# vga-group/tauray

Hardware: AMD Instinct MI355X
Metric: Mray/s (closest-hit + shadow rays traced) @1920x1080, 4 bounces, 1 spp (higher is better)
Workload: dtype f32

## Files before the change

tauray_amd/csrc/api.hip:

```cpp
#include <cstdlib>
#include <cstring>
#include <mutex>
#include <string>
#include <vector>

#include "pt.h"
#include "trace.h"
#include "trace_quad.h"
#include "specialize.h"
#include "tonemap.h"
#include "../../include/tauray_image.hh"
#include "../../include/tauray_exr.hh"

namespace tr {

static thread_local std::string g_error;
int set_error(const std::string& msg) { g_error = msg; return 1; }

#define HIPCHK(x) do { hipError_t e_ = (x); if (e_ != hipSuccess) return set_error(std::string(#x) + ": " + hipGetErrorString(e_)); } while (0)

namespace {

constexpr int KB = TR_BLOCK;

// ... 119 lines not shown
                if (lh.light >= 0) out[ri] = HitRecord{-1, lh.light, lh.t, 0.0f, lh.t};
            }
        }
    }
    if (overflow) *overflow_flag = 1;
}
__global__ __launch_bounds__(KB) void k_query_terminal(SceneView sv, uint n, const float* rays, const uint* seeds, const uint* fallback, HitRecord* out, uint* overflow_flag,
                                                       int* qspill) {
    __shared__ int s_stack_rows[TR_STACK_WORDS];
    int* const s_stack = s_stack_rows + TR_STACK_ROW0;
    __shared__ int s_owner[(KB / 64) * TR_OWNER_WORDS];
    int* my_stack = s_stack + threadIdx.x;
    QuadCtx qc;
    qc.wave_stack = s_stack + (threadIdx.x & ~63u);
    qc.owner_tab = s_owner + (threadIdx.x >> 6) * TR_OWNER_WORDS;
    qc.spill = qspill + ((size_t)blockIdx.x * (KB / 64) + (threadIdx.x >> 6)) * (16u * TR_QSPILL);
    int overflow = 0;
    TraceStats st = {};
    for (uint base = blockIdx.x * KB; base < n; base += gridDim.x * KB) {
        const uint i = base + threadIdx.x;
        const bool valid = i < n;
        float r[8] = {0, 0, 0, 0, 0, 0, 0, 0};
        if (valid) for (int k = 0; k < 8; ++k) r[k] = rays[(size_t)i * 8 + k];
        const uint seed = (valid && seeds) ? seeds[i] : 0u;
        TerminalRay term = {valid && !(fallback && fallback[i] != 0u), false};
        HitRecord hit;
        if (seeds) trace_closest_wave4<0, false, false, true>(sv, valid, F3(r[0], r[1], r[2]), F3(r[4], r[5], r[6]), r[3], r[7], seed, my_stack, qc, hit, st, overflow, &term);
        else trace_closest_wave4<1, false, false, true>(sv, valid, F3(r[0], r[1], r[2]), F3(r[4], r[5], r[6]), r[3], r[7], 0u, my_stack, qc, hit, st, overflow, &term);
        if (valid) out[i] = term.blocked ? HitRecord{TR_HIT_BLOCKED, -1, 0.0f, 0.0f, -1.0f} : hit;
    }
    if (overflow) *overflow_flag = 1;
}
template <bool TWO_LEVEL>
__global__ __launch_bounds__(KB) void k_query_shadow(SceneView sv, uint n, const float* rays, float* out, uint* overflow_flag) {
    __shared__ int s_stack_rows[TR_STACK_WORDS];
    int* const s_stack = s_stack_rows + TR_STACK_ROW0;
    int overflow = 0;
    TraceStats st = {};
    for (uint i = blockIdx.x * KB + threadIdx.x; i < n; i += gridDim.x * KB) {
        const float* r = rays + (size_t)i * 8;
        out[i] = trace_shadow4<false, TWO_LEVEL>(sv, F3(r[0], r[1], r[2]), F3(r[4], r[5], r[6]), r[3], r[7], s_stack + threadIdx.x, st, overflow);
    }
    if (overflow) *overflow_flag = 1;
}

__global__ __launch_bounds__(KB) void k_stitch(LaunchCtx L, const f4* partial, uint pw, uint ph, f4* primary, uint viewports, float blend_ratio) {
    uint per_view = L.strategy == 2 ? L.launch_w : pw * ph;
    uint i = blockIdx.x * KB + threadIdx.x;
    if (i >= per_view * viewports) return;
    uint z = i / per_view, p = i % per_view;
    uint sx, sy, ox, oy;
    if (L.strategy == 2) {
        uint j = permute_region_id(L.index + p, L.size_x, L.size_y, L.count);
        if (j >= L.size_x * L.size_y) return;
        sx = p % L.size_x; sy = p / L.size_x;
        ox = j % L.size_x; oy = j / L.size_x;
    } else {
        sx = p % pw; sy = p / pw;
        ox = sx; oy = sy * L.count + L.index;
        if (oy >= L.size_y) return;
    }
    f4 c = partial[((size_t)z * ph + sy) * pw + sx];
    size_t o = ((size_t)z * L.size_y + oy) * L.size_x + ox;
    if (blend_ratio < 1.0f) c = mix4(primary[o], c, blend_ratio);
    primary[o] = c;
}

#define TR_STITCH_BATCH 15
struct StitchBatch { LaunchCtx L[TR_STITCH_BATCH]; const f4* partial[TR_STITCH_BATCH]; uint pw[TR_STITCH_BATCH], ph[TR_STITCH_BATCH]; };
__global__ __launch_bounds__(KB) void k_stitch_batch(StitchBatch B, f4* primary, uint viewports, float blend_ratio) {
    const uint e = blockIdx.y;
    const LaunchCtx L = B.L[e];
    const uint pw = B.pw[e], ph = B.ph[e];
    const f4* partial = B.partial[e];
// ... 14 lines not shown
    }
    f4 c = partial[((size_t)z * ph + sy) * pw + sx];
    size_t o = ((size_t)z * L.size_y + oy) * L.size_x + ox;
    if (blend_ratio < 1.0f) c = mix4(primary[o], c, blend_ratio);
    primary[o] = c;
}

__global__ __launch_bounds__(KB) void k_tonemap(const f4* in, f4* out, uint w, uint h, uint layers, int op, float exposure, float gamma, int grid) {
    size_t i = (size_t)blockIdx.x * KB + threadIdx.x;
    size_t n = (size_t)w * h * layers;
    if (i >= n) return;
    out[i] = tonemap_pixel(in[i], op, exposure, gamma, grid, (uint)(i % w), (uint)((i / w) % h));
}

template <typename T>
int upload_array(T*& dst, const void* src, size_t count) {
    dst = nullptr;
    if (count == 0 || !src) return 0;
    HIPCHK(hipMalloc(&dst, count * sizeof(T)));
    HIPCHK(hipMemcpy(dst, src, count * sizeof(T), hipMemcpyHostToDevice));
    return 0;
}

}
}

using namespace tr;

struct trhip_device {
    int hip_device = 0;
    DeviceScene scene;
    uint* overflow_flag = nullptr;
    int* qspill = nullptr;
};
constexpr uint QUERY_BLOCKS = 2048;
struct trhip_pt {
    trhip_device* dev;
    PtStage* stage;
};

namespace tr { int device_index(const trhip_device* dev) { return dev ? dev->hip_device : -1; } }
namespace tr { DeviceScene* device_scene(trhip_device* dev) { return dev ? &dev->scene : nullptr; } }
namespace tr { uint* device_overflow_flag(trhip_device* dev) { return dev ? dev->overflow_flag : nullptr; } }

#define DEVCHK(dev) do { if (!(dev)) return set_error("null trhip_device"); hipError_t e_ = hipSetDevice((dev)->hip_device); \
    if (e_ != hipSuccess) return set_error(std::string("hipSetDevice: ") + hipGetErrorString(e_)); } while (0)

extern "C" {

const char* trhip_last_error(void) { return g_error.c_str(); }

int trhip_image_decode(const void* data, size_t bytes, uint32_t* width, uint32_t* height, uint32_t* channels_in_file, uint8_t** rgba_out) {
    if (!data || !width || !height || !rgba_out) return set_error("trhip_image_decode: null argument");
    try {
        tr::image::decoded d = tr::image::decode(static_cast<const uint8_t*>(data), bytes);
        uint8_t* p = static_cast<uint8_t*>(malloc(d.rgba.size() ? d.rgba.size() : 1));
        if (!p) return set_error("trhip_image_decode: out of memory");
        memcpy(p, d.rgba.data(), d.rgba.size());
        *width = d.w; *height = d.h; *rgba_out = p;
        if (channels_in_file) *channels_in_file = (uint32_t)d.channels_in_file;
    } catch (const std::exception& e) { return set_error(e.what()); }
    return 0;
}
int trhip_image_decode_texels(const void* data, size_t bytes, uint32_t* width, uint32_t* height, uint32_t* channels_in_file, uint32_t* bits, uint8_t** texels_out) {
    if (!data || !width || !height || !bits || !texels_out) return set_error("trhip_image_decode_texels: null argument");
    try {
// ... 28 lines not shown
    try {
        const std::vector<uint8_t> b = tr::exr::encode(rgba, width, height, alpha != 0, half != 0, compression);
        uint8_t* p = static_cast<uint8_t*>(malloc(b.size()));
        if (!p) return set_error("trhip_exr_encode: out of memory");
        memcpy(p, b.data(), b.size());
        *bytes_out = p; *size_out = b.size();
    } catch (const std::exception& e) { return set_error(e.what()); }
    return 0;
}
void trhip_exr_free(void* p) { free(p); }

int trhip_device_create(int hip_device, trhip_device** out) {
    if (!out) return set_error("trhip_device_create: null out");
    int count = 0;
    hipError_t e = hipGetDeviceCount(&count);
    if (e != hipSuccess || count == 0) return set_error(std::string("trhip_device_create: no HIP device available (") + hipGetErrorString(e) + ")");
    if (hip_device < 0 || hip_device >= count) return set_error("trhip_device_create: device index out of range");
    HIPCHK(hipSetDevice(hip_device));
    trhip_device* d = new trhip_device();
    d->hip_device = hip_device;
    HIPCHK(hipMalloc(&d->overflow_flag, 4));
    HIPCHK(hipMemset(d->overflow_flag, 0, 4));
    { int cls = -1; (void)stream_pool_class(nullptr, &cls, true); }
    *out = d;
    return 0;
}
void trhip_device_destroy(trhip_device* dev) {
    if (!dev) return;
    (void)hipSetDevice(dev->hip_device);
    (void)hipDeviceSynchronize();
    dev->scene.free_all();
    if (dev->overflow_flag) (void)hipFree(dev->overflow_flag);
    if (dev->qspill) (void)hipFree(dev->qspill);
    delete dev;
}
int trhip_malloc(trhip_device* dev, size_t bytes, void** out) { DEVCHK(dev); HIPCHK(hipMalloc(out, bytes ? bytes : 16)); return 0; }
int trhip_free(trhip_device* dev, void* ptr) { DEVCHK(dev); if (ptr) HIPCHK(hipFree(ptr)); return 0; }
int trhip_upload(trhip_device* dev, void* dst, const void* src, size_t bytes, void* stream) {
    DEVCHK(dev); HIPCHK(hipMemcpyAsync(dst, src, bytes, hipMemcpyHostToDevice, (hipStream_t)stream)); HIPCHK(hipStreamSynchronize((hipStream_t)stream)); return 0;
}
int trhip_download(trhip_device* dev, void* dst, const void* src, size_t bytes, void* stream) {
    DEVCHK(dev); HIPCHK(hipMemcpyAsync(dst, src, bytes, hipMemcpyDeviceToHost, (hipStream_t)stream)); HIPCHK(hipStreamSynchronize((hipStream_t)stream)); return 0;
}
int trhip_memset(trhip_device* dev, void* dst, int value, size_t bytes, void* stream) { DEVCHK(dev); HIPCHK(hipMemsetAsync(dst, value, bytes, (hipStream_t)stream)); return 0; }
int trhip_sync(trhip_device* dev, void* stream) { DEVCHK(dev); HIPCHK(hipStreamSynchronize((hipStream_t)stream)); return 0; }
int trhip_stream_create(trhip_device* dev, void** stream_out) {
    DEVCHK(dev);
    if (!stream_out) return set_error("trhip_stream_create: null argument");
    hipStream_t st = nullptr;
    if (int rc = stream_pool_acquire(&st)) return rc;
    *stream_out = st;
    return 0;
}
int trhip_stream_destroy(trhip_device* dev, void* stream) {
    DEVCHK(dev);
    if (stream) { HIPCHK(hipStreamSynchronize((hipStream_t)stream)); stream_pool_release((hipStream_t)stream); }
    return 0;
}
int trhip_stream_pipe_class(trhip_device* dev, void* stream, int32_t* pipe_class_out) {
    DEVCHK(dev);
    if (!pipe_class_out) return set_error("trhip_stream_pipe_class: null argument");
    int c = -1;
    if (int rc = stream_pool_class((hipStream_t)stream, &c, true)) return rc;
    *pipe_class_out = c;
    return 0;
}
// ... 560 lines not shown
    HIPCHK(hipGetLastError());
    return 0;
}

int trhip_trace_closest(trhip_device* dev, uint32_t n, const void* rays_dev, const void* seeds_dev, int include_lights, void* hits_dev, void* stream) {
    DEVCHK(dev);
    if (!dev->scene.accel_built) return set_error("trhip_trace_closest: call trhip_scene_build_accel first");
    if (n == 0) return 0;
    uint blocks = std::min((n + KB - 1) / KB, QUERY_BLOCKS);
    if (!dev->qspill) HIPCHK(hipMalloc(&dev->qspill, (size_t)QUERY_BLOCKS * (KB / 64) * 16u * TR_QSPILL * sizeof(int)));
    hipLaunchKernelGGL(dev->scene.two_level ? k_query_closest<true> : k_query_closest<false>, dim3(blocks), dim3(KB), 0, (hipStream_t)stream, dev->scene.view(), n, (const float*)rays_dev,
                       (const uint*)seeds_dev, include_lights, (HitRecord*)hits_dev, dev->overflow_flag, dev->qspill);
    HIPCHK(hipGetLastError());
    return 0;
}
int trhip_trace_terminal(trhip_device* dev, uint32_t n, const void* rays_dev, const void* seeds_dev, const void* fallback_dev, void* hits_dev, void* stream) {
    DEVCHK(dev);
    const DeviceScene& s = dev->scene;
    if (!s.accel_built) return set_error("trhip_trace_terminal: call trhip_scene_build_accel first");
    if (s.two_level || !s.tris) return set_error("trhip_trace_terminal: the terminal query walks an all-merged structure");
    if (s.emitter_count > TR_EMITTER_MAX) return set_error("trhip_trace_terminal: " + std::to_string(s.emitter_count) + " emitter triangles, the query tests at most " + std::to_string(TR_EMITTER_MAX));
    if (n == 0) return 0;
    uint blocks = std::min((n + KB - 1) / KB, QUERY_BLOCKS);
    if (!dev->qspill) HIPCHK(hipMalloc(&dev->qspill, (size_t)QUERY_BLOCKS * (KB / 64) * 16u * TR_QSPILL * sizeof(int)));
    hipLaunchKernelGGL(k_query_terminal, dim3(blocks), dim3(KB), 0, (hipStream_t)stream, s.view(), n, (const float*)rays_dev, (const uint*)seeds_dev, (const uint*)fallback_dev,
                       (HitRecord*)hits_dev, dev->overflow_flag, dev->qspill);
    HIPCHK(hipGetLastError());
    return 0;
}
int trhip_trace_shadow(trhip_device* dev, uint32_t n, const void* rays_dev, void* visibility_dev, void* stream) {
    DEVCHK(dev);
    if (!dev->scene.accel_built) return set_error("trhip_trace_shadow: call trhip_scene_build_accel first");
    if (n == 0) return 0;
    uint blocks = std::min((n + KB - 1) / KB, 2048u);
    hipLaunchKernelGGL(dev->scene.two_level ? k_query_shadow<true> : k_query_shadow<false>, dim3(blocks), dim3(KB), 0, (hipStream_t)stream, dev->scene.view(), n, (const float*)rays_dev,
                       (float*)visibility_dev, dev->overflow_flag);
    HIPCHK(hipGetLastError());
    return 0;
}

int trhip_stitch(trhip_device* dev, const trhip_distribution* pd, const void* partial_dev, uint32_t pw, uint32_t ph, void* primary_dev,
                 uint32_t viewports, float blend_ratio, void* stream) {
    DEVCHK(dev);
    if (!pd || pd->strategy == 0) return set_error("trhip_stitch: needs a scanline or shuffled-strips partial");
    LaunchCtx L = make_launch(*pd);
    size_t per_view = pd->strategy == 2 ? L.launch_w : (size_t)pw * ph;
    size_t n = per_view * viewports;
    if (n == 0) return 0;
    hipLaunchKernelGGL(k_stitch, dim3((uint)((n + KB - 1) / KB)), dim3(KB), 0, (hipStream_t)stream, L, (const f4*)partial_dev, pw, ph,
                       (f4*)primary_dev, viewports, blend_ratio);
    HIPCHK(hipGetLastError());
    return 0;
}

int trhip_stitch_batch(trhip_device* dev, uint32_t count, const trhip_distribution* pds, const void* const* partials_dev, const uint32_t* pws,
                       const uint32_t* phs, void* primary_dev, uint32_t viewports, float blend_ratio, void* stream) {
    DEVCHK(dev);
    if (count == 0) return 0;
    if (!pds || !partials_dev || !pws || !phs) return set_error("trhip_stitch_batch: null argument");
    for (uint32_t first = 0; first < count; first += TR_STITCH_BATCH) {
        const uint32_t m = std::min<uint32_t>(TR_STITCH_BATCH, count - first);
        StitchBatch B{};
        size_t n_max = 0;
        for (uint32_t k = 0; k < m; ++k) {
            const trhip_distribution& pd = pds[first + k];
            if (pd.strategy == 0) return set_error("trhip_stitch_batch: needs scanline or shuffled-strips partials");
            B.L[k] = make_launch(pd);
            B.partial[k] = (const f4*)partials_dev[first + k]; B.pw[k] = pws[first + k]; B.ph[k] = phs[first + k];
            const size_t per_view = pd.strategy == 2 ? B.L[k].launch_w : (size_t)B.pw[k] * B.ph[k];
// ... 25 lines not shown
```

tauray_amd/csrc/bvh_build.hip:

```cpp
#include <algorithm>
#include <cctype>
#include <chrono>
#include <cmath>
#include <map>
#include <tuple>
#include <vector>
#include "build.h"

#include <rocprim/rocprim.hpp>

namespace tr {

namespace {

constexpr int BT = 256;

TR_DEV uint float_flip(float f) { uint u = __float_as_uint(f); return (u & 0x80000000u) ? ~u : (u | 0x80000000u); }
TR_HD float float_unflip(uint u) {
    uint v = (u & 0x80000000u) ? (u & 0x7FFFFFFFu) : ~u;
    float f;
#if defined(__HIP_DEVICE_COMPILE__)
    f = __uint_as_float(v);
#else
    memcpy(&f, &v, 4);
// ... 658 lines not shown
    uint i = blockIdx.x * BT + threadIdx.x;
    if (i >= count) return;
    const Bvh4Node& nd = nodes4[level[i]];
    for (int c = 0; c < 4; ++c) {
        const int ch = nd.child[c];
        if (ch >= 0 && ch != 0x7FFFFFFF) next[atomicAdd(next_count, 1u)] = (uint)ch;
    }
}

__global__ __launch_bounds__(BT) void k_refit_level(uint count, const uint* level, Bvh4Node* nodes4, const TriRecord* tris, float* node_bounds) {
    uint i = blockIdx.x * BT + threadIdx.x;
    if (i >= count) return;
    const uint id = level[i];
    Bvh4Node nd = nodes4[id];
    float lo[3] = {__builtin_huge_valf(), __builtin_huge_valf(), __builtin_huge_valf()};
    float hi[3] = {-__builtin_huge_valf(), -__builtin_huge_valf(), -__builtin_huge_valf()};
    for (int c = 0; c < 4; ++c) {
        const int ch = nd.child[c];
        if (ch == 0x7FFFFFFF) continue;
        float blo[3], bhi[3];
        if (ch < 0) {
            const TriRecord& t = tris[~ch];
            for (int k = 0; k < 3; ++k) { blo[k] = fminf(fminf(t.v0[k], t.v1[k]), t.v2[k]); bhi[k] = fmaxf(fmaxf(t.v0[k], t.v1[k]), t.v2[k]); }
        } else {
            for (int k = 0; k < 3; ++k) { blo[k] = node_bounds[6 * (size_t)ch + k]; bhi[k] = node_bounds[6 * (size_t)ch + 3 + k]; }
        }
        nd.lox[c] = blo[0]; nd.loy[c] = blo[1]; nd.loz[c] = blo[2]; nd.hix[c] = bhi[0]; nd.hiy[c] = bhi[1]; nd.hiz[c] = bhi[2];
        for (int k = 0; k < 3; ++k) { lo[k] = fminf(lo[k], blo[k]); hi[k] = fmaxf(hi[k], bhi[k]); }
    }
    nodes4[id] = nd;
    for (int k = 0; k < 3; ++k) { node_bounds[6 * (size_t)id + k] = lo[k]; node_bounds[6 * (size_t)id + 3 + k] = hi[k]; }
}

static int refit_two_level(DeviceScene& ds, hipStream_t stream, trhip_accel_info* info);
int refit_accel(DeviceScene& ds, hipStream_t stream, trhip_accel_info* info) {
    if (ds.two_level) {
        if (ds.accel_tri_count != ds.tri_count || ds.tlas_capacity != ds.tlas_leaf_count)
            return set_error("trhip_scene_refit_accel: no acceleration structure to refit; call trhip_scene_build_accel first");
        return refit_two_level(ds, stream, info);
    }
    const uint n = ds.leaf_count;
    if (ds.accel_tri_count != ds.tri_count || ds.accel_capacity == 0xFFFFFFFFu || (n > 0 && !ds.tris) || (n > 1 && !ds.nodes4))
        return set_error("trhip_scene_refit_accel: no acceleration structure to refit; call trhip_scene_build_accel first");
    hipEvent_t e0, e1;
    HIPCHK(hipEventCreate(&e0)); HIPCHK(hipEventCreate(&e1));
    HIPCHK(hipEventRecord(e0, stream));
    SceneView sv = ds.view();
    const uint n1 = ds.node_count;
    if (n1 > 0 && !ds.levels_valid) {
        if (!ds.level_nodes) HIPCHK(hipMalloc(&ds.level_nodes, (size_t)n1 * 4));
        if (!ds.node_bounds) HIPCHK(hipMalloc(&ds.node_bounds, (size_t)n1 * 24));
        uint* counter = nullptr;
        HIPCHK(hipMalloc(&counter, 4));
        const uint root = 0;
        HIPCHK(hipMemcpyAsync(ds.level_nodes, &root, 4, hipMemcpyHostToDevice, stream));
        ds.level_offsets.assign(1, 0u);
        uint begin = 0, count = 1;
        while (count > 0) {
            ds.level_offsets.push_back(begin + count);
            if (begin + count >= n1) break;
            HIPCHK(hipMemsetAsync(counter, 0, 4, stream));
            hipLaunchKernelGGL(k_expand_level, dim3((count + BT - 1) / BT), dim3(BT), 0, stream, count, ds.level_nodes + begin, ds.nodes4,
                               ds.level_nodes + begin + count, counter);
            uint next = 0;
            HIPCHK(hipMemcpyAsync(&next, counter, 4, hipMemcpyDeviceToHost, stream));
            HIPCHK(hipStreamSynchronize(stream));
            begin += count; count = next;
            if (ds.level_offsets.size() > 4096) { (void)hipFree(counter); return set_error("trhip_scene_refit_accel: hierarchy too deep"); }
        }
        (void)hipFree(counter);
        ds.levels_valid = true;
        if (getenv("TRHIP_DEBUG"))
            fprintf(stderr, "[trhip] 4-wide tree: %u live nodes of %u slots in %zu levels, %.3f children per node\n", ds.level_offsets.back(), n1,
                    ds.level_offsets.size() - 1, (double)(n + ds.level_offsets.back() - 1) / (double)ds.level_offsets.back());
    }
    if (n > 0) hipLaunchKernelGGL(k_retransform, dim3((n + BT - 1) / BT), dim3(BT), 0, stream, sv, n, ds.tris, ds.alpha_base, ds.alpha_tris);
    for (size_t l = ds.level_offsets.size(); l-- > 1;) {
        const uint lo = ds.level_offsets[l - 1], cnt = ds.level_offsets[l] - lo;
        if (cnt) hipLaunchKernelGGL(k_refit_level, dim3((cnt + BT - 1) / BT), dim3(BT), 0, stream, cnt, ds.level_nodes + lo, ds.nodes4, ds.tris, ds.node_bounds);
    }
    HIPCHK(hipGetLastError());
    ds.accel_built = true;
    if (ds.gather_emissive_triangles && ds.host_tri_light_count > 0 && ds.tri_lights) {
        HIPCHK(hipMemsetAsync(ds.tri_lights, 0, (size_t)ds.host_tri_light_count * sizeof(TriLight), stream));
        SceneView sv2 = ds.view();
        hipLaunchKernelGGL(k_extract_tri_lights, dim3((ds.tri_count + BT - 1) / BT), dim3(BT), 0, stream, sv2, ds.tri_prefix, ds.tri_lights);
    }
    if (int rc = gather_emitters(ds, stream)) return rc;
    HIPCHK(hipEventRecord(e1, stream));
    HIPCHK(hipEventSynchronize(e1));
    float ms = 0;
    HIPCHK(hipEventElapsedTime(&ms, e0, e1));
    (void)hipEventDestroy(e0); (void)hipEventDestroy(e1);
    ds.layout.blas_updated = 1; ds.layout.blas_ms = ms;
    if (info) {
        memset(info, 0, sizeof(*info));
        info->triangle_count = ds.tri_count; info->leaf_count = n; info->node_count = ds.node_count; info->node_bytes = 112u; info->tri_light_count = ds.tri_light_count;
        info->build_ms = ms;
        for (int k = 0; k < 3; ++k) { info->bounds_min[k] = ds.bounds_lo[k]; info->bounds_max[k] = ds.bounds_hi[k]; }
    }
    return 0;
}

struct TreePlan {
    size_t sort_bytes = 0, scan_bytes = 0;
    size_t o_cbounds, o_unsorted, o_keys, o_keys_sorted, o_vals, o_vals_sorted, o_leaf_box, o_sort, o_children, o_sizes, o_parent, o_parent_leaf,
           o_node_box, o_arrive, o_cref0, o_cref1, o_cbox0, o_cbox1, o_nn, o_valid, o_pos, o_scan, o_new_id, o_nodes2;
    size_t o_uparent, o_moves, o_lock, o_optstat, o_ccost, o_cdec;
    char* base = nullptr;
    uint* cbounds() const { return reinterpret_cast<uint*>(base + o_cbounds); }
    TriRecord* unsorted() const { return reinterpret_cast<TriRecord*>(base + o_unsorted); }
};

// ... 167 lines not shown
    return 0;
}

static int build_two_level(DeviceScene& ds, hipStream_t stream, trhip_accel_info* info);
static int refit_two_level(DeviceScene& ds, hipStream_t stream, trhip_accel_info* info);

int build_accel(DeviceScene& ds, hipStream_t stream, trhip_accel_info* info) {
    if (ds.accel_strategy != TRHIP_AS_ALL_MERGED) return build_two_level(ds, stream, info);
    const uint n_scene = ds.tri_count;
    hipEvent_t e0, e1;
    HIPCHK(hipEventCreate(&e0)); HIPCHK(hipEventCreate(&e1));
    HIPCHK(hipEventRecord(e0, stream));
    ds.accel_built = false;
    ds.levels_valid = false;
    SceneView sv = ds.view();
    sv.tri_count = n_scene;
    const uint n_tri = n_scene;
    const uint n_cap = n_tri;
    uint n = n_tri;
    const size_t n1 = n_cap > 1 ? n_cap - 1 : 0;
    if (ds.two_level) ds.free_accel();
    TreePlan P;
    if (int rc = plan_tree(ds, stream, n_cap, P)) return rc;
    uint* cbounds = P.cbounds();
    {
        const uint init[32] = {0xFFFFFFFFu, 0xFFFFFFFFu, 0xFFFFFFFFu, 0, 0, 0, 0, 0, 0, 0, 0, 0, 0, 0, 0, 0, 0xFFFFFFFFu, 0xFFFFFFFFu, 0xFFFFFFFFu, 0, 0, 0, 0, 0, 0, 0, 0, 0, 0, 0, 0, 0};
        HIPCHK(hipMemcpyAsync(cbounds, init, sizeof(init), hipMemcpyHostToDevice, stream));
    }
    if (ds.accel_capacity != n_cap) {
        ds.free_accel();
        if (n_cap > 0) HIPCHK(hipMalloc(&ds.tris, (size_t)n_cap * sizeof(TriRecord) + sizeof(EmitterSet)));
        if (n1 > 0) {
            if ((uint64_t)n1 * sizeof(Bvh4Node) > 0xFFFFFFFFull) return set_error("trhip_scene_build_accel: more than 2^25 nodes");
            HIPCHK(hipMalloc(&ds.nodes4, n1 * sizeof(Bvh4Node)));
        }
        ds.accel_capacity = n_cap;
    }
    if (n_tri > 0) {
        TriRecord* unsorted = P.unsorted();
        const uint tblocks = (n_tri + BT - 1) / BT;
        hipLaunchKernelGGL(k_pretransform, dim3(tblocks < 1024u ? tblocks : 1024u), dim3(BT), 0, stream, sv, ds.tri_prefix, ds.non_opaque, ds.alpha_base, ds.alpha_tris, unsorted, cbounds);
    }
    if (int rc = build_tree(ds, stream, P, n, ds.tris, ds.nodes4)) return rc;
    ds.leaf_count = n;
    ds.node_count = n > 1 ? n - 1 : 0;
    ds.accel_tri_count = n_tri;
    ds.accel_built = true;
    ds.tri_light_count = 0;
    if (ds.gather_emissive_triangles && ds.host_tri_light_count > 0) {
        if (!ds.tri_lights) HIPCHK(hipMalloc(&ds.tri_lights, (size_t)ds.host_tri_light_count * sizeof(TriLight)));
        HIPCHK(hipMemsetAsync(ds.tri_lights, 0, (size_t)ds.host_tri_light_count * sizeof(TriLight), stream));
        ds.tri_light_count = ds.host_tri_light_count;
        SceneView sv2 = ds.view();
        hipLaunchKernelGGL(k_extract_tri_lights, dim3((n_tri + BT - 1) / BT), dim3(BT), 0, stream, sv2, ds.tri_prefix, ds.tri_lights);
        HIPCHK(hipGetLastError());
    }
    if (int rc = gather_emitters(ds, stream)) return rc;
    HIPCHK(hipEventRecord(e1, stream));
    HIPCHK(hipEventSynchronize(e1));
    float ms = 0;
    HIPCHK(hipEventElapsedTime(&ms, e0, e1));
    (void)hipEventDestroy(e0); (void)hipEventDestroy(e1);
    uint hb[6];
    HIPCHK(hipMemcpy(hb, cbounds, sizeof(hb), hipMemcpyDeviceToHost));
    for (int k = 0; k < 3; ++k) { ds.bounds_lo[k] = float_unflip(hb[k]); ds.bounds_hi[k] = float_unflip(hb[3 + k]); }
    ds.layout = {};
    ds.layout.strategy = TRHIP_AS_ALL_MERGED; ds.layout.blas_count = 1; ds.layout.blas_updated = 1;
    ds.layout.node_bytes = (uint64_t)ds.node_count * sizeof(Bvh4Node); ds.layout.record_bytes = (uint64_t)n * sizeof(TriRecord);
    ds.layout.blas_ms = ms;
    if (info) {
        info->triangle_count = n_tri;
        info->leaf_count = n;
        info->node_count = ds.node_count;
        info->node_bytes = 112u;
        info->tri_light_count = ds.tri_light_count;
        info->build_ms = ms;
        for (int k = 0; k < 3; ++k) { info->bounds_min[k] = float_unflip(hb[k]); info->bounds_max[k] = float_unflip(hb[3 + k]); }
    }
    return 0;
}
// ... 645 lines not shown
```

tauray_amd/csrc/common.h:

```cpp
#pragma once
#include <hip/hip_runtime.h>
#include <hip/hip_fp16.h>
#include <stdint.h>
#include <string.h>
#include <cstring>

#include "../../include/trhip.h"

#define TR_DEV __device__ __forceinline__
#define TR_HD __host__ __device__ __forceinline__

namespace tr {

typedef uint32_t uint;

struct f2 { float x, y; };
struct f3 { float x, y, z; };
struct f4 { float x, y, z, w; };
struct u4 { uint x, y, z, w; };
struct u2 { uint x, y; };

TR_HD f2 F2(float a, float b) { return {a, b}; }
TR_HD f2 F2(float a) { return {a, a}; }
TR_HD f3 F3(float a, float b, float c) { return {a, b, c}; }
// ... 85 lines not shown
    m4 model, model_normal, model_prev; Material mat;
};
struct DirectionalLight { f3 color; int shadow_map_index; f3 dir; float dir_cutoff; };
struct PointLight {
    f3 color, dir, pos; float radius, dir_cutoff, dir_falloff, cutoff_radius, spot_radius;
    int shadow_map_index, padding;
};
struct TriLight { f3 pos[3]; uint emission_factor, instance_id, primitive_id; uint uv[3]; int emission_tex_id; };
struct AliasEntry { uint alias_id, probability; float pdf, alias_pdf; };
struct CameraData { m4 view, view_inverse, view_proj, proj_inverse; f4 origin, dof_params, projection_info, pan; };
struct MeshSpan { uint vertex_offset, vertex_count, index_offset, triangle_count; };
struct ShadeTri { f3 pos[3]; f3 normal[3]; f2 uv[3]; float pad[8]; };
struct Skin { uint joints[4]; float weights[4]; };
struct TextureInfo { uint width, height, texel_offset, format; };
enum { TEXTURE_FORMAT_RGBA8 = 0, TEXTURE_FORMAT_RGBA16 = 1 };
#pragma pack(pop)
static_assert(sizeof(Vertex) == 48 && sizeof(Material) == 80 && sizeof(Instance) == 288 && sizeof(ShadeTri) == 128, "layout");
static_assert(sizeof(DirectionalLight) == 32 && sizeof(PointLight) == 64 && sizeof(TriLight) == 64, "layout");
static_assert(sizeof(CameraData) == 320 && sizeof(AliasEntry) == 16, "layout");

struct alignas(64) BvhNode {
    float lo0[3], hi0[3], lo1[3], hi1[3];
    int child0, child1;
    uint pad0, pad1;
};
static_assert(sizeof(BvhNode) == 64, "node layout");

struct alignas(128) Bvh4Node {
    float lox[4], hix[4], loy[4], hiy[4], loz[4], hiz[4];
    int child[4];
    int pad[4];
};
static_assert(sizeof(Bvh4Node) == 128, "Bvh4Node layout");

struct alignas(16) TriRecord {
    float v0[3], v1[3], v2[3];
    uint inst_flags, prim, alpha;
};
static_assert(sizeof(TriRecord) == 48, "tri layout");
struct alignas(16) AlphaTri { f2 uv0, uv1, uv2; float factor; int tex; };
static_assert(sizeof(AlphaTri) == 32, "alpha record layout");

struct HitRecord { int instance_id, primitive_id; float u, v, t; };

#define TR_INST_FROM_RECORD 0xFFFFFFFFu
#define TR_TLAS_IDENTITY 1u
struct alignas(64) TlasLeaf {
    float xf[12];
    int blas_root;
    uint inst_word;
    uint alpha_base;
    uint flags;
};
static_assert(sizeof(TlasLeaf) == 64, "TLAS leaf layout");

struct SceneView {
    const Instance* instances;
    const MeshSpan* spans;
    const Vertex* vertices;
    const uint* indices;
    const PointLight* point_lights;
    const DirectionalLight* directional_lights;
    const TriLight* tri_lights;
    const TextureInfo* tex_infos;
    const uint8_t* texels;
    const f4* envmap;
    const AliasEntry* alias_table;
    const CameraData* cameras;
    const CameraData* prev_cameras;
    const MeshSpan* obj_spans;
    const Vertex* obj_vertices;
    const ShadeTri* shade_tris;
    const f4* shade_tangents;
    const TriRecord* tris;
    const AlphaTri* alpha_tris;
    const Bvh4Node* nodes4;
    f4 environment_factor;
    int environment_proj;
    uint instance_count, point_light_count, directional_light_count, tri_light_count;
    uint env_w, env_h;
    uint tri_count, node_count;
    uint wide_textures;
};
TR_HD const TlasLeaf* tlas_leaves(const SceneView& sv) { return reinterpret_cast<const TlasLeaf*>(sv.nodes4 + sv.node_count); }

#define TR_LIGHT_KAPPA 0.001953125f
struct alignas(16) LightTreeHeader { uint use_tree, node_count, leaf_count, pad; };
static_assert(sizeof(LightTreeHeader) == 16, "light tree header layout");
TR_HD size_t light_tree_node_offset(uint point_light_count) { return ((size_t)point_light_count * sizeof(PointLight) + sizeof(LightTreeHeader) + 127) & ~(size_t)127; }
TR_HD size_t light_allocation_bytes(uint point_light_count) {
    return light_tree_node_offset(point_light_count) + (size_t)(point_light_count > 1 ? point_light_count - 1 : 1) * sizeof(Bvh4Node);
}
TR_HD const LightTreeHeader* light_tree_header(const SceneView& sv) { return reinterpret_cast<const LightTreeHeader*>(sv.point_lights + sv.point_light_count); }
TR_HD const Bvh4Node* light_tree_nodes(const SceneView& sv) {
    return reinterpret_cast<const Bvh4Node*>(reinterpret_cast<const char*>(sv.point_lights) + light_tree_node_offset(sv.point_light_count));
}


#define TR_EMITTER_MAX 16
struct alignas(16) EmitterSet { float planes[24]; uint count, pad[3]; uint index[TR_EMITTER_MAX]; };
static_assert(sizeof(EmitterSet) == 176 && sizeof(TriRecord) % 16 == 0, "emitter set layout");
TR_HD const EmitterSet* emitter_set(const SceneView& sv) { return reinterpret_cast<const EmitterSet*>(sv.tris + sv.tri_count); }

}
```

tauray_amd/csrc/trace_quad.h:

```cpp
#pragma once
#include "trace.h"

namespace tr {

#ifndef TR_QUAD_SWITCH
#define TR_QUAD_SWITCH 16
#endif
#ifndef TR_QUAD_VOTE
#define TR_QUAD_VOTE 4
#endif
#ifndef TR_TERMINAL_SLOT_ORDER
#define TR_TERMINAL_SLOT_ORDER 1
#endif
#ifndef TR_TERMINAL_QUADS
#define TR_TERMINAL_QUADS 1
#endif
#define TR_QSPILL TR_SPILL_STACK
static_assert(TR_QUAD_SWITCH <= 16, "a wave has sixteen quads");

#define TR_OWNER_WORDS 16

struct QuadCtx {
    int* wave_stack;
    int* owner_tab;
    int* spill;
    TL(uint* tl;)
};

template <int CTRL> TR_DEV int quad_perm(int v) { return __builtin_amdgcn_update_dpp(0, v, CTRL, 0xF, 0xF, true); }
TR_DEV int qrot1(int v) { return quad_perm<0x39>(v); }
TR_DEV int qrot2(int v) { return quad_perm<0x4E>(v); }
TR_DEV int qrot3(int v) { return quad_perm<0x93>(v); }
TR_DEV float qrot1f(float v) { return __int_as_float(qrot1(__float_as_int(v))); }
TR_DEV float qrot2f(float v) { return __int_as_float(qrot2(__float_as_int(v))); }
TR_DEV int bperm(int byte_addr, int v) { return __builtin_amdgcn_ds_bpermute(byte_addr, v); }
TR_DEV float bpermf(int byte_addr, float v) { return __int_as_float(__builtin_amdgcn_ds_bpermute(byte_addr, __float_as_int(v))); }

TR_DEV int quad_lane() {
    int l;
    asm volatile("v_mbcnt_lo_u32_b32 %0, -1, 0\n\tv_mbcnt_hi_u32_b32 %0, -1, %0" : "=v"(l));
    return l & 3;
}

TR_DEV void wave_sync_lds() {
    __builtin_amdgcn_fence(__ATOMIC_RELEASE, "workgroup");
    __builtin_amdgcn_wave_barrier();
    __builtin_amdgcn_fence(__ATOMIC_ACQUIRE, "workgroup");
}

struct QuadRay {
    RayPre r;
    float tmin;
};

TR_DEV int quad_child_box(const QuadRay& r, const Bvh4Node* nodes, int node, int q, float tmax, bool& hit, float& t0 TL(, TlPhase* tlp = nullptr)) {
    float nx, fx, ny, fy, nz, fz;
    int c;
    {
        const char* base = reinterpret_cast<const char*>(nodes);
        const uint t = ((uint)node << 7) | ((uint)q << 2);
        const uint ax = t | r.r.nkx, ay = t | r.r.nky, az = t | r.r.nkz;
        nx = *reinterpret_cast<const float*>(base + (size_t)ax); fx = *reinterpret_cast<const float*>(base + (size_t)(ax ^ 16u));
        ny = *reinterpret_cast<const float*>(base + (size_t)ay); fy = *reinterpret_cast<const float*>(base + (size_t)(ay ^ 16u));
        nz = *reinterpret_cast<const float*>(base + (size_t)az); fz = *reinterpret_cast<const float*>(base + (size_t)(az ^ 16u));
        c = *reinterpret_cast<const int*>(base + (size_t)t + 96);
        TL(if (tlp) tlp->loads_issued();)
    }
    const float tx0 = (nx - r.r.op.x) * r.r.ip.x, tx1 = (fx - r.r.op.x) * r.r.ip.x;
    const float ty0 = (ny - r.r.op.y) * r.r.ip.y, ty1 = (fy - r.r.op.y) * r.r.ip.y;
    const float tz0 = (nz - r.r.op.z) * r.r.ip.z, tz1 = (fz - r.r.op.z) * r.r.ip.z;
    t0 = fmaxf(fmaxf(tx0, ty0), fmaxf(tz0, r.tmin));
    const float t1 = fminf(fminf(fminf(tx1, ty1), tz1), tmax) * TR_SLAB_PAD;
    hit = t0 <= t1;
    asm volatile("" : "+v"(c));
    return c;
}

struct QuadStack {
    int* lds;
    int* glob;
    int sp;
    int overflow;
    TR_DEV void store(int pos, int v) {
        if (pos < TR_LDS_STACK) lds[pos * TR_BLOCK] = v;
        else {
            const int k = pos - TR_LDS_STACK;
            if (k >= TR_QSPILL) overflow++;
            glob[k < TR_QSPILL ? k : TR_QSPILL - 1] = v;
            __builtin_amdgcn_fence(__ATOMIC_RELEASE, "workgroup");
        }
    }
    TR_DEV int load(int pos) {
        int v = lds[(pos < TR_LDS_STACK ? pos : 0) * TR_BLOCK];
        asm volatile("" : "+v"(v));
        if (pos >= TR_LDS_STACK) {
            __builtin_amdgcn_fence(__ATOMIC_ACQUIRE, "workgroup");
            const int k = pos - TR_LDS_STACK;
            v = glob[k < TR_QSPILL ? k : TR_QSPILL - 1];
        }
        return v;
    }
};

struct QuadDeal {
    int q, qd;
    int my_rank;
    int src, back;
    bool has_ray;
};
TR_DEV QuadDeal quad_deal(unsigned long long act, bool live, const RayPre& r, float tmin, int node, const LaneStack& stk, const int* spill, const QuadCtx& qc,
                          int& overflow, QuadRay& qr, QuadStack& qs, int& qnode) {
    QuadDeal d;
    const int lane = threadIdx.x & 63, n_act = __popcll(act);
    d.q = lane & 3; d.qd = lane >> 2;
    d.my_rank = __popcll(act & ((1ull << lane) - 1ull));
    if (live) {
        qc.owner_tab[d.my_rank] = lane;
        for (int e = TR_LDS_STACK; e < stk.sp; ++e) {
            const int k = e - TR_LDS_STACK;
            if (k < TR_QSPILL) qc.spill[d.my_rank * TR_QSPILL + k] = spill[k < TR_SPILL_STACK ? k : TR_SPILL_STACK - 1];
            else overflow++;
        }
    }
    wave_sync_lds();
    d.has_ray = d.qd < n_act;
    const int owner = d.has_ray ? qc.owner_tab[d.qd] : lane;
    d.src = owner << 2;
    d.back = d.my_rank << 4;
    const int src = d.src;
    qr.r.op = F3(bpermf(src, r.op.x), bpermf(src, r.op.y), bpermf(src, r.op.z));
    qr.r.ip = F3(bpermf(src, r.ip.x), bpermf(src, r.ip.y), bpermf(src, r.ip.z));
    qr.r.Sx = bpermf(src, r.Sx); qr.r.Sy = bpermf(src, r.Sy);
    const uint packed = (uint)bperm(src, (int)(r.nkx | (r.nky << 8) | (r.nkz << 16)));
    qr.r.nkx = packed & 0xFFu; qr.r.nky = (packed >> 8) & 0xFFu; qr.r.nkz = (packed >> 16) & 0xFFu;
    qr.tmin = bpermf(src, tmin);
    qnode = bperm(src, node);
    qs.lds = qc.wave_stack + owner;
    qs.glob = qc.spill + d.qd * TR_QSPILL;
    qs.sp = bperm(src, stk.sp);
    qs.overflow = 0;
    return d;
}

TR_DEV void quad_descend(bool inner, uint key, int c, QuadStack& qs, int& qnode, bool& qlive) {
    const uint k1 = (uint)qrot1((int)key), k2 = (uint)qrot2((int)key), k3 = (uint)qrot3((int)key);
    const int rank = (int)(k1 < key) + (int)(k2 < key) + (int)(k3 < key);
    int n_inner = inner ? 1 : 0;
    n_inner += qrot1(n_inner); n_inner += qrot2(n_inner);
    int nx = (inner && rank == 0) ? c : 0;
    nx |= qrot1(nx); nx |= qrot2(nx);
    if (n_inner > 0) {
        if (inner && rank >= 1) qs.store(qs.sp + n_inner - 1 - rank, c);
        qs.sp += n_inner - 1;
        qnode = nx;
    } else if (qs.sp == 0) qlive = false;
    else { qs.sp--; qnode = qs.load(qs.sp); }
}

TR_DEV void quad_inherited_leaf(int q, int& pend, QuadStack& qs, int& qnode, bool& qlive) {
    if (q == 0) pend = ~qnode;
    if (qs.sp == 0) qlive = false;
    else { qs.sp--; qnode = qs.load(qs.sp); }
}

template <int ALPHA_MODE, bool COUNT, bool TWO_LEVEL = false, bool TERMINAL = false>
TR_DEV void trace_closest_wave4(const SceneView& sv, bool valid, f3 org, f3 dir, float tmin, float tmax, uint seed,
                                int* lds_stack, const QuadCtx& qc, HitRecord& hit, TraceStats& st, int& overflow, TerminalRay* term = nullptr) {
// ... 160 lines not shown
                    TL(TlPhase tlp; const int tl_units = __popcll(__ballot(true)); tlp.begin();)
                    TriHit tr;
                    if (COUNT) st.tris++;
                    if (tri_intersect(qr.r, sv.tris, (uint)pend, qr.tmin, __builtin_huge_valf(), tr TL(, &tlp))) {
                        const float t = tr.t, bu = tr.bu, bv = tr.bv;
                        const uint inst = tr.inst_flags & 0x7FFFFFFFu;
                        bool accept = t < lt || (t == lt && linst != 0xFFFFFFFFu && (inst < linst || (inst == linst && tr.prim < lprim)));
                        if (accept && (tr.inst_flags & 0x80000000u)) {
                            if (COUNT) st.alpha++;
                            const float a = candidate_alpha(sv, tr.alpha, bu, bv);
                            const float cutoff = ALPHA_MODE == 0 ? alpha_cutoff_hash(qseed, (int)inst, (int)tr.prim) : 0.0001f;
                            accept = !(a <= cutoff);
                        }
                        lt = accept ? t : lt; lu = accept ? bu : lu; lv = accept ? bv : lv;
                        linst = accept ? inst : linst; lprim = accept ? tr.prim : lprim;
                        if constexpr (TERMINAL) took = accept;
                    }
                    TL(tlp.end(qc.tl, TL_QT, tl_units, (tl_units - 1) >> 3, -1);)
                }
                pend = -1;
                if constexpr (TERMINAL) {
                    int z = took ? 1 : 0;
                    z |= qrot1(z); z |= qrot2(z);
                    if (z != 0 && qearly) { qblocked = true; qlive = false; }
                }
                float m = lt;
                m = fminf(m, qrot1f(m)); m = fminf(m, qrot2f(m));
                qbest = fminf(qbest, m);
            } else if (can_node && qnode < 0) quad_inherited_leaf(quad_lane(), pend, qs, qnode, qlive);
            else if (can_node) {
                bool hitb; float t0;
                TL(TlPhase tlp; const int tl_units = __popcll(__ballot(true)) >> 2; tlp.begin();)
                const int q = quad_lane();
                const int c = quad_child_box(qr, sv.nodes4, qnode, q, qbest, hitb, t0 TL(, &tlp));
                if (COUNT && q == 0) st.nodes++;
                const bool inner = hitb && c >= 0;
                if (hitb && c < 0) pend = ~c;
                quad_descend(inner, inner ? ((__float_as_uint(t0) & ~3u) | (uint)q) : 0xFFFFFFFFu, c, qs, qnode, qlive);
                if (COUNT) st.maxsp = max(st.maxsp, (uint)qs.sp);
                TL(tlp.end(qc.tl, TL_QN, tl_units, (tl_units - 1) >> 1, TL_QN_WAIT_HIST);)
            }
        }
        {
            float ot = qrot1f(lt), ou = qrot1f(lu), ov = qrot1f(lv); uint oi = (uint)qrot1((int)linst), op = (uint)qrot1((int)lprim);
            bool take = ot < lt || (ot == lt && (oi < linst || (oi == linst && op < lprim)));
            lt = take ? ot : lt; lu = take ? ou : lu; lv = take ? ov : lv; linst = take ? oi : linst; lprim = take ? op : lprim;
            ot = qrot2f(lt); ou = qrot2f(lu); ov = qrot2f(lv); oi = (uint)qrot2((int)linst); op = (uint)qrot2((int)lprim);
            take = ot < lt || (ot == lt && (oi < linst || (oi == linst && op < lprim)));
            lt = take ? ot : lt; lu = take ? ou : lu; lv = take ? ov : lv; linst = take ? oi : linst; lprim = take ? op : lprim;
        }
        int qo = qs.overflow;
        qo += qrot1(qo); qo += qrot2(qo);
        const int back = deal.back;
        const float rt = bpermf(back, lt), ru = bpermf(back, lu), rv = bpermf(back, lv);
        const uint ri = (uint)bperm(back, (int)linst), rp = (uint)bperm(back, (int)lprim);
        const int ro = bperm(back, qo);
        if (live) { best_t = rt; best_u = ru; best_v = rv; best_inst = ri; best_prim = rp; overflow += ro; }
        if constexpr (TERMINAL) {
            const int rb = bperm(back, qblocked ? 1 : 0);
            if (live) blocked = blocked || rb != 0;
        }
    }
    if constexpr (TERMINAL) term->blocked = blocked;
    overflow += stk.overflow ? 1 : 0;
    TL(tl_misc(qc.tl, 0, 1); tl_misc(qc.tl, 1, tl_now() - tl_enter); tl_misc(qc.tl, 4, tl_wall() - tl_wall0);)

    bool found = best_inst != 0xFFFFFFFFu;
// ... 63 lines not shown
        const int q = deal.q, src = deal.src;
        const float qtmax = bpermf(src, tmax);
        const float owner_vis = bpermf(src, visibility);
        float lvis = q == 0 ? owner_vis : 1.0f;
        bool qlive = deal.has_ray;
        int pend = -1;
        while (true) {
            int w = pend >= 0 ? 1 : 0;
            w |= qrot1(w); w |= qrot2(w);
            const bool qwait = w != 0;
            if (__ballot(qlive || qwait) == 0) break;
            const bool can_node = qlive && !qwait;
            const bool tri_phase = __popcll(__ballot(pend >= 0)) >= TR_QUAD_VOTE || __ballot(can_node) == 0;
            if (tri_phase) {
                if (pend >= 0) {
                    TriHit tr;
                    if (COUNT) st.tris++;
                    if (tri_intersect(qr.r, sv.tris, (uint)pend, qr.tmin, qtmax, tr)) {
                        if (!(tr.inst_flags & 0x80000000u)) lvis = 0.0f;
                        else {
                            if (COUNT) st.alpha++;
                            lvis *= 1.0f - candidate_alpha(sv, tr.alpha, tr.bu, tr.bv);
                        }
                    }
                }
                pend = -1;
                int z = lvis == 0.0f ? 1 : 0;
                z |= qrot1(z); z |= qrot2(z);
                if (z) qlive = false;
            } else if (can_node && qnode < 0) quad_inherited_leaf(quad_lane(), pend, qs, qnode, qlive);
            else if (can_node) {
                bool hitb; float t0;
                const int q = quad_lane();
                const int c = quad_child_box(qr, sv.nodes4, qnode, q, qtmax, hitb, t0);
                if (COUNT && q == 0) st.nodes++;
                const bool inner = hitb && c >= 0;
                if (hitb && c < 0) pend = ~c;
                quad_descend(inner, inner ? (uint)q : 0xFFFFFFFFu, c, qs, qnode, qlive);
            }
        }
        float v = lvis;
        v *= qrot1f(v); v *= qrot2f(v);
        int qo = qs.overflow;
        qo += qrot1(qo); qo += qrot2(qo);
        const int back = deal.back;
        const float rv = bpermf(back, v);
        const int ro = bperm(back, qo);
        if (live) { visibility = rv; overflow += ro; }
    }
    overflow += stk.overflow ? 1 : 0;
    return visibility;
}

}
```

Measured before the change: 3939.

## Add child-major BVH4 node copy and route shadow queries through wave4 quad traversal

The BVH build and refit now also write a child-major copy of each BVH4 node, placed right after the existing node array, which is allocated twice as large. In that copy each child's bounds and reference sit together in 32 bytes, so a quad lane fetches its child box with two 16-byte vector loads instead of seven scattered scalar loads. The lane then picks near and far planes by ray-direction sign, using a per-axis origin and inverse direction stored in QuadRay. Separately, the standalone shadow query kernel switches from per-thread traversal to the cooperative wave4 quad traversal, backed by a new spill buffer and owner table. The costs are double the node memory, an extra derive kernel on every build or refit, and possible overlap with TLAS leaf storage, which uses the same offset after the node array.

New measurement: 3896. 1.1% lower.

```diff
diff --git a/tauray_amd/csrc/api.hip b/tauray_amd/csrc/api.hip
--- a/tauray_amd/csrc/api.hip
+++ b/tauray_amd/csrc/api.hip
@@ -175,14 +175,23 @@
     if (overflow) *overflow_flag = 1;
 }
 template <bool TWO_LEVEL>
-__global__ __launch_bounds__(KB) void k_query_shadow(SceneView sv, uint n, const float* rays, float* out, uint* overflow_flag) {
+__global__ __launch_bounds__(KB) void k_query_shadow(SceneView sv, uint n, const float* rays, float* out, uint* overflow_flag, int* qspill) {
     __shared__ int s_stack_rows[TR_STACK_WORDS];
     int* const s_stack = s_stack_rows + TR_STACK_ROW0;
+    __shared__ int s_owner[(KB / 64) * TR_OWNER_WORDS];
+    QuadCtx qc;
+    qc.wave_stack = s_stack + (threadIdx.x & ~63u);
+    qc.owner_tab = s_owner + (threadIdx.x >> 6) * TR_OWNER_WORDS;
+    qc.spill = qspill + ((size_t)blockIdx.x * (KB / 64) + (threadIdx.x >> 6)) * (16u * TR_QSPILL);
     int overflow = 0;
     TraceStats st = {};
-    for (uint i = blockIdx.x * KB + threadIdx.x; i < n; i += gridDim.x * KB) {
-        const float* r = rays + (size_t)i * 8;
-        out[i] = trace_shadow4<false, TWO_LEVEL>(sv, F3(r[0], r[1], r[2]), F3(r[4], r[5], r[6]), r[3], r[7], s_stack + threadIdx.x, st, overflow);
+    for (uint base = blockIdx.x * KB; base < n; base += gridDim.x * KB) {
+        const uint i = base + threadIdx.x;
+        const bool valid = i < n;
+        float r[8] = {0, 0, 0, 0, 0, 0, 0, 0};
+        if (valid) for (int k = 0; k < 8; ++k) r[k] = rays[(size_t)i * 8 + k];
+        const float vis = trace_shadow_wave4<false, TWO_LEVEL>(sv, valid, F3(r[0], r[1], r[2]), F3(r[4], r[5], r[6]), r[3], r[7], s_stack + threadIdx.x, qc, st, overflow);
+        if (valid) out[i] = vis;
     }
     if (overflow) *overflow_flag = 1;
 }
@@ -263,6 +272,7 @@
     DeviceScene scene;
     uint* overflow_flag = nullptr;
     int* qspill = nullptr;
+    int* qspill_shadow = nullptr;
 };
 constexpr uint QUERY_BLOCKS = 2048;
 struct trhip_pt {
@@ -357,6 +367,7 @@
     dev->scene.free_all();
     if (dev->overflow_flag) (void)hipFree(dev->overflow_flag);
     if (dev->qspill) (void)hipFree(dev->qspill);
+    if (dev->qspill_shadow) (void)hipFree(dev->qspill_shadow);
     delete dev;
 }
 int trhip_malloc(trhip_device* dev, size_t bytes, void** out) { DEVCHK(dev); HIPCHK(hipMalloc(out, bytes ? bytes : 16)); return 0; }
@@ -983,9 +994,10 @@
     DEVCHK(dev);
     if (!dev->scene.accel_built) return set_error("trhip_trace_shadow: call trhip_scene_build_accel first");
     if (n == 0) return 0;
-    uint blocks = std::min((n + KB - 1) / KB, 2048u);
+    uint blocks = std::min((n + KB - 1) / KB, QUERY_BLOCKS);
+    if (!dev->qspill_shadow) HIPCHK(hipMalloc(&dev->qspill_shadow, (size_t)QUERY_BLOCKS * (KB / 64) * 16u * TR_QSPILL * sizeof(int)));
     hipLaunchKernelGGL(dev->scene.two_level ? k_query_shadow<true> : k_query_shadow<false>, dim3(blocks), dim3(KB), 0, (hipStream_t)stream, dev->scene.view(), n, (const float*)rays_dev,
-                       (float*)visibility_dev, dev->overflow_flag);
+                       (float*)visibility_dev, dev->overflow_flag, dev->qspill_shadow);
     HIPCHK(hipGetLastError());
     return 0;
 }
diff --git a/tauray_amd/csrc/bvh_build.hip b/tauray_amd/csrc/bvh_build.hip
--- a/tauray_amd/csrc/bvh_build.hip
+++ b/tauray_amd/csrc/bvh_build.hip
@@ -714,6 +714,23 @@
     for (int k = 0; k < 3; ++k) { node_bounds[6 * (size_t)id + k] = lo[k]; node_bounds[6 * (size_t)id + 3 + k] = hi[k]; }
 }
 
+__global__ __launch_bounds__(BT) void k_child_major(uint count, const Bvh4Node* nodes4, Bvh4ChildNode* out) {
+    const uint i = blockIdx.x * BT + threadIdx.x;
+    if (i >= count * 4u) return;
+    const Bvh4Node& nd = nodes4[i >> 2];
+    const uint c = i & 3u;
+    Bvh4Child k;
+    k.lo[0] = nd.lox[c]; k.lo[1] = nd.loy[c]; k.lo[2] = nd.loz[c]; k.ref = nd.child[c];
+    k.hi[0] = nd.hix[c]; k.hi[1] = nd.hiy[c]; k.hi[2] = nd.hiz[c]; k.pad = 0u;
+    out[i >> 2].child[c] = k;
+}
+static void derive_child_major(DeviceScene& ds, hipStream_t stream) {
+    const uint n1 = ds.node_count;
+    if (n1 == 0) return;
+    const uint blocks = (uint)(((size_t)n1 * 4 + BT - 1) / BT);
+    hipLaunchKernelGGL(k_child_major, dim3(blocks), dim3(BT), 0, stream, n1, ds.nodes4, reinterpret_cast<Bvh4ChildNode*>(ds.nodes4 + n1));
+}
+
 static int refit_two_level(DeviceScene& ds, hipStream_t stream, trhip_accel_info* info);
 int refit_accel(DeviceScene& ds, hipStream_t stream, trhip_accel_info* info) {
     if (ds.two_level) {
@@ -761,6 +778,7 @@
         const uint lo = ds.level_offsets[l - 1], cnt = ds.level_offsets[l] - lo;
         if (cnt) hipLaunchKernelGGL(k_refit_level, dim3((cnt + BT - 1) / BT), dim3(BT), 0, stream, cnt, ds.level_nodes + lo, ds.nodes4, ds.tris, ds.node_bounds);
     }
+    derive_child_major(ds, stream);
     HIPCHK(hipGetLastError());
     ds.accel_built = true;
     if (ds.gather_emissive_triangles && ds.host_tri_light_count > 0 && ds.tri_lights) {
@@ -994,7 +1012,7 @@
         if (n_cap > 0) HIPCHK(hipMalloc(&ds.tris, (size_t)n_cap * sizeof(TriRecord) + sizeof(EmitterSet)));
         if (n1 > 0) {
             if ((uint64_t)n1 * sizeof(Bvh4Node) > 0xFFFFFFFFull) return set_error("trhip_scene_build_accel: more than 2^25 nodes");
-            HIPCHK(hipMalloc(&ds.nodes4, n1 * sizeof(Bvh4Node)));
+            HIPCHK(hipMalloc(&ds.nodes4, 2 * n1 * sizeof(Bvh4Node)));
         }
         ds.accel_capacity = n_cap;
     }
@@ -1008,6 +1026,7 @@
     ds.node_count = n > 1 ? n - 1 : 0;
     ds.accel_tri_count = n_tri;
     ds.accel_built = true;
+    derive_child_major(ds, stream);
     ds.tri_light_count = 0;
     if (ds.gather_emissive_triangles && ds.host_tri_light_count > 0) {
         if (!ds.tri_lights) HIPCHK(hipMalloc(&ds.tri_lights, (size_t)ds.host_tri_light_count * sizeof(TriLight)));
diff --git a/tauray_amd/csrc/common.h b/tauray_amd/csrc/common.h
--- a/tauray_amd/csrc/common.h
+++ b/tauray_amd/csrc/common.h
@@ -141,6 +141,10 @@
     int pad[4];
 };
 static_assert(sizeof(Bvh4Node) == 128, "Bvh4Node layout");
+
+struct alignas(32) Bvh4Child { float lo[3]; int ref; float hi[3]; uint pad; };
+struct alignas(128) Bvh4ChildNode { Bvh4Child child[4]; };
+static_assert(sizeof(Bvh4Child) == 32 && sizeof(Bvh4ChildNode) == 128, "Bvh4ChildNode layout");
 
 struct alignas(16) TriRecord {
     float v0[3], v1[3], v2[3];
@@ -192,6 +196,7 @@
     uint wide_textures;
 };
 TR_HD const TlasLeaf* tlas_leaves(const SceneView& sv) { return reinterpret_cast<const TlasLeaf*>(sv.nodes4 + sv.node_count); }
+TR_HD const Bvh4ChildNode* child_major_nodes(const SceneView& sv) { return reinterpret_cast<const Bvh4ChildNode*>(sv.nodes4 + sv.node_count); }
 
 #define TR_LIGHT_KAPPA 0.001953125f
 struct alignas(16) LightTreeHeader { uint use_tree, node_count, leaf_count, pad; };
diff --git a/tauray_amd/csrc/trace_quad.h b/tauray_amd/csrc/trace_quad.h
--- a/tauray_amd/csrc/trace_quad.h
+++ b/tauray_amd/csrc/trace_quad.h
@@ -50,25 +50,24 @@
 
 struct QuadRay {
     RayPre r;
+    f3 o, i;
     float tmin;
 };
-
-TR_DEV int quad_child_box(const QuadRay& r, const Bvh4Node* nodes, int node, int q, float tmax, bool& hit, float& t0 TL(, TlPhase* tlp = nullptr)) {
-    float nx, fx, ny, fy, nz, fz;
-    int c;
-    {
-        const char* base = reinterpret_cast<const char*>(nodes);
-        const uint t = ((uint)node << 7) | ((uint)q << 2);
-        const uint ax = t | r.r.nkx, ay = t | r.r.nky, az = t | r.r.nkz;
-        nx = *reinterpret_cast<const float*>(base + (size_t)ax); fx = *reinterpret_cast<const float*>(base + (size_t)(ax ^ 16u));
-        ny = *reinterpret_cast<const float*>(base + (size_t)ay); fy = *reinterpret_cast<const float*>(base + (size_t)(ay ^ 16u));
-        nz = *reinterpret_cast<const float*>(base + (size_t)az); fz = *reinterpret_cast<const float*>(base + (size_t)(az ^ 16u));
-        c = *reinterpret_cast<const int*>(base + (size_t)t + 96);
-        TL(if (tlp) tlp->loads_issued();)
-    }
-    const float tx0 = (nx - r.r.op.x) * r.r.ip.x, tx1 = (fx - r.r.op.x) * r.r.ip.x;
-    const float ty0 = (ny - r.r.op.y) * r.r.ip.y, ty1 = (fy - r.r.op.y) * r.r.ip.y;
-    const float tz0 = (nz - r.r.op.z) * r.r.ip.z, tz1 = (fz - r.r.op.z) * r.r.ip.z;
+TR_DEV float ray_axis(f3 v, uint kx, uint ky, uint axis) { return kx == axis ? v.x : (ky == axis ? v.y : v.z); }
+
+TR_DEV int quad_child_box(const QuadRay& r, const Bvh4ChildNode* nodes, int node, int q, float tmax, bool& hit, float& t0 TL(, TlPhase* tlp = nullptr)) {
+    const char* base = reinterpret_cast<const char*>(nodes);
+    const uint t = ((uint)node << 7) | ((uint)q << 5);
+    const f4 lo = *reinterpret_cast<const f4*>(base + (size_t)t), hi = *reinterpret_cast<const f4*>(base + (size_t)(t | 16u));
+    TL(if (tlp) tlp->loads_issued();)
+    int c = __float_as_int(lo.w);
+    const bool sx = __float_as_int(r.i.x) < 0, sy = __float_as_int(r.i.y) < 0, sz = __float_as_int(r.i.z) < 0;
+    const float nx = sx ? hi.x : lo.x, fx = sx ? lo.x : hi.x;
+    const float ny = sy ? hi.y : lo.y, fy = sy ? lo.y : hi.y;
+    const float nz = sz ? hi.z : lo.z, fz = sz ? lo.z : hi.z;
+    const float tx0 = (nx - r.o.x) * r.i.x, tx1 = (fx - r.o.x) * r.i.x;
+    const float ty0 = (ny - r.o.y) * r.i.y, ty1 = (fy - r.o.y) * r.i.y;
+    const float tz0 = (nz - r.o.z) * r.i.z, tz1 = (fz - r.o.z) * r.i.z;
     t0 = fmaxf(fmaxf(tx0, ty0), fmaxf(tz0, r.tmin));
     const float t1 = fminf(fminf(fminf(tx1, ty1), tz1), tmax) * TR_SLAB_PAD;
     hit = t0 <= t1;
@@ -133,6 +132,11 @@
     qr.r.Sx = bpermf(src, r.Sx); qr.r.Sy = bpermf(src, r.Sy);
     const uint packed = (uint)bperm(src, (int)(r.nkx | (r.nky << 8) | (r.nkz << 16)));
     qr.r.nkx = packed & 0xFFu; qr.r.nky = (packed >> 8) & 0xFFu; qr.r.nkz = (packed >> 16) & 0xFFu;
+    {
+        const uint kx = qr.r.nkx >> 5, ky = qr.r.nky >> 5;
+        qr.o = F3(ray_axis(qr.r.op, kx, ky, 0u), ray_axis(qr.r.op, kx, ky, 1u), ray_axis(qr.r.op, kx, ky, 2u));
+        qr.i = F3(ray_axis(qr.r.ip, kx, ky, 0u), ray_axis(qr.r.ip, kx, ky, 1u), ray_axis(qr.r.ip, kx, ky, 2u));
+    }
     qr.tmin = bpermf(src, tmin);
     qnode = bperm(src, node);
     qs.lds = qc.wave_stack + owner;
@@ -359,7 +363,7 @@
                 bool hitb; float t0;
                 TL(TlPhase tlp; const int tl_units = __popcll(__ballot(true)) >> 2; tlp.begin();)
                 const int q = quad_lane();
-                const int c = quad_child_box(qr, sv.nodes4, qnode, q, qbest, hitb, t0 TL(, &tlp));
+                const int c = quad_child_box(qr, child_major_nodes(sv), qnode, q, qbest, hitb, t0 TL(, &tlp));
                 if (COUNT && q == 0) st.nodes++;
                 const bool inner = hitb && c >= 0;
                 if (hitb && c < 0) pend = ~c;
@@ -489,7 +493,7 @@
             else if (can_node) {
                 bool hitb; float t0;
                 const int q = quad_lane();
-                const int c = quad_child_box(qr, sv.nodes4, qnode, q, qtmax, hitb, t0);
+                const int c = quad_child_box(qr, child_major_nodes(sv), qnode, q, qtmax, hitb, t0);
                 if (COUNT && q == 0) st.nodes++;
                 const bool inner = hitb && c >= 0;
                 if (hitb && c < 0) pend = ~c;
```
